# harryjfowen/PointsToWood

Measured on AMD Instinct MI355X. Metric: classified points/sec, higher is better.
Workload: dtype f16x3

## Files before the change

### include/p2w.h

```cpp
#ifndef P2W_H
#define P2W_H

#include <stddef.h>
#include <stdint.h>

#ifdef __cplusplus
extern "C" {
#endif

typedef void* p2w_stream_t;

#define P2W_OK 0
#define P2W_EINVAL (-1)
#define P2W_ENULL (-2)
#define P2W_EALIGN (-3)
#define P2W_EWORKSPACE (-4)
#define P2W_EUNSUPPORTED (-5)

#define P2W_MAX_K 64
#define P2W_MAX_K_WIDE 100
#define P2W_MAX_K_CONV 32

int32_t p2w_version(void);
const char* p2w_strerror(int32_t code);
// ... 170 lines not shown
    float* m;
    float* v;
    int64_t n;
} p2w_optim_tensor;
typedef struct p2w_optim_hyper {
    double lr, beta1, beta2, eps, weight_decay, max_norm, growth_factor, backoff_factor;
    int32_t growth_interval;
    int32_t scaling;
} p2w_optim_hyper;
typedef struct p2w_optim_state {
    double sumsq;
    float norm, coef;
    float inv_scale;
    float scale;
    int32_t found_inf;
    int32_t growth_tracker;
    int64_t t;
    int64_t skipped;
    float decay, omb1, beta2, omb2, step_size, rsb2, eps;
    int32_t reserved;
} p2w_optim_state;
size_t p2w_clip_adamw_ws_size(const int64_t* numel, int32_t T);
int32_t p2w_clip_adamw(const p2w_optim_tensor* tensors, int32_t T, const p2w_optim_hyper* hyper, p2w_optim_state* state, void* ws,
                       size_t ws_bytes, p2w_stream_t stream);

int32_t p2w_vote(const int32_t* nbr, const int32_t* deg, int32_t k, const float* pred, const float* prob, int32_t n,
                 float any_wood, float* label_out, float* pwood_out, p2w_stream_t stream);

int32_t p2w_tile_bbox(const float* xyzr, const int32_t* ptr, int32_t B, int32_t n_bound, float* bbox, p2w_stream_t stream);
int32_t p2w_tile_bbox_count(int32_t B, int32_t n_bound);


int32_t p2w_stem(const float* xyzr, int32_t n, const float* w, const float* b, int32_t C, float* out,
                 p2w_stream_t stream);

typedef struct p2w_epilogue {
    const float* bias;
    const float* sc0;
    const float* sh0;
    const float* sc1;
    const float* sh1;
    const float* residual;
    int32_t ldr;
    int32_t relu0, relu1, relu2, relu_final;
    uint32_t* range;
    const void* interp;
    int32_t interp_rows;
} p2w_epilogue;

#define P2W_RANGE_HI 6.0e4f
#define P2W_RANGE_LO 0.03125f
#define P2W_RANGE_SLOTS 16
#define P2W_RANGE_WORDS (64 * P2W_RANGE_SLOTS)

void p2w_packed_dims(int32_t N, int32_t K, int32_t* N_pad, int32_t* K_pad);

int32_t p2w_gemm(const float* A, int32_t lda, const float* Wp, int32_t M, int32_t N, int32_t K,
                 const p2w_epilogue* epi, float* out, int32_t ldo, p2w_stream_t stream);

int32_t p2w_sa_conv(const float* P, int32_t ldp, const float* xyzr_src, const int32_t* idx, const int32_t* batch_dst,
                    const float* sf, const int32_t* nbr, const int32_t* deg, int32_t kw, int32_t M,
                    const float* w1r4 , const float* W2p, int32_t C1, int32_t C2,
                    const float* b2, const float* bn_s, const float* bn_t, float* out, int32_t ldo,
                    p2w_stream_t stream);

#define P2W_PREC_F16X3 0
#define P2W_PREC_F16 1
#define P2W_PREC_BF16 2
int32_t p2w_packed_dims_h(int32_t prec, int32_t N, int32_t K, int32_t* N_pad, int32_t* K_pad);

#define P2W_GEMM_TILE_128 1
#define P2W_GEMM_TILE_256 2
#define P2W_GEMM_GENERIC_EPI 4
#define P2W_GEMM_ORDER_ROWS 8
#define P2W_GEMM_ORDER_COLS 16
#define P2W_GEMM_RESIDUAL_H 32
#define P2W_GEMM_STREAMK 64
#define P2W_GEMM_NO_STREAMK 128
#define P2W_GEMM_TILE_64 (1 << 24)
#define P2W_GEMM_NO_TILE_64 (1 << 25)
#define P2W_SA_ITEM_256 1
#define P2W_SA_ITEM_128 2
#define P2W_SA_PACK8 4

int32_t p2w_gemm_h2(int32_t prec, const void* A_h, int32_t ldh_a, const void* Wh, float wscale, int32_t M, int32_t N,
                    int32_t K, const p2w_epilogue* epi, float* out_f32, int32_t ldo, void* out_h, int32_t ldh_o,
                    int32_t flags, p2w_stream_t stream);
size_t p2w_gemm_h2_sk_ws_bytes(void);
int32_t p2w_gemm_h2_sk(int32_t prec, const void* A_h, int32_t ldh_a, const void* Wh, float wscale, int32_t M, int32_t N,
                       int32_t K, const p2w_epilogue* epi, float* out_f32, int32_t ldo, void* out_h, int32_t ldh_o,
                       void* ws, size_t ws_bytes, int32_t flags, p2w_stream_t stream);
size_t p2w_gemm_h2_rowdot_ws_bytes(int32_t M, int32_t N);
int32_t p2w_gemm_h2_rowdot(int32_t prec, const void* A_h, int32_t ldh_a, const void* Wh, float wscale, int32_t M, int32_t N,
                           int32_t K, const p2w_epilogue* epi, const float* dot_w, float dot_b, float* out, void* ws,
                           size_t ws_bytes, int32_t flags, p2w_stream_t stream);
size_t p2w_sa_conv_h_ws_bytes(int32_t M, int32_t flags);
int32_t p2w_sa_conv_h(int32_t prec, const float* P, int32_t ldp, int32_t n_src, const float* xyzr_src, const int32_t* idx,
                      const int32_t* batch_dst, const float* sf, const int32_t* nbr, const int32_t* deg, int32_t kw,
                      int32_t M, const float* w1r4, const void* W2h, float wscale, int32_t C1, int32_t C2,
                      const float* b2, const float* bn_s, const float* bn_t, float* out, int32_t ldo, void* out_h,
                      int32_t ldh, void* ws, size_t ws_bytes, int32_t flags, p2w_stream_t stream);
int32_t p2w_sa_conv_h_rows(int32_t prec, const float* P, int32_t ldp, int32_t n_src, const float* xyzr_src, const int32_t* idx,
                           const int32_t* batch_dst, const float* sf, const int32_t* nbr, const int32_t* deg, int32_t kw,
                           int32_t M, const float* w1r4, const void* W2h, float wscale, int32_t C1, int32_t C2,
                           const float* b2, const float* bn_s, const float* bn_t, float* out, int32_t ldo, void* out_h,
                           int32_t ldh, void* ws, size_t ws_bytes, int32_t flags, const int32_t* src_row, uint32_t* range,
                           p2w_stream_t stream);
int32_t p2w_stem_h2(int32_t prec, const float* xyzr, int32_t n, const float* w, const float* b, int32_t C, float* out,
                    void* out_h, int32_t ldh, uint32_t* range, p2w_stream_t stream);
int32_t p2w_stem_h2_indexed(int32_t prec, const float* xyzr, int32_t n, const float* w, const float* b, int32_t C, float* out,
                            void* out_h, int32_t ldh, uint32_t* range, p2w_stream_t stream);
int32_t p2w_interp_concat_h2(int32_t prec, const float* xc, int32_t Fc, const float* xyzr_c, const float* xyzr_f,
                             const int32_t* nbr, const int32_t* deg, int32_t kw, const float* skip, int32_t Fs, int32_t m,
                             void* out_h, int32_t ldh, p2w_stream_t stream);
int32_t p2w_interp_weights(const float* xyzr_c, const float* xyzr_f, const int32_t* nbr, const int32_t* deg, int32_t kw, int32_t m,
                           void* records, p2w_stream_t stream);
int32_t p2w_concat_xyz_h2(int32_t prec, const float* x, int32_t F, const float* xyzr, int32_t m, void* out_h, int32_t ldh,
                          p2w_stream_t stream);

int32_t p2w_interp_concat(const float* xc, int32_t Fc, const float* xyzr_c, const float* xyzr_f, const int32_t* nbr,
                          const int32_t* deg, int32_t kw, const float* skip, int32_t Fs, int32_t m, float* out,
                          int32_t ldo, p2w_stream_t stream);

int32_t p2w_concat_xyz(const float* x, int32_t F, const float* xyzr, int32_t m, float* out, int32_t ldo,
                       p2w_stream_t stream);

int32_t p2w_segment_max(const float* x, int32_t ldx, int32_t F, const int32_t* ptr, int32_t B, float* out,
                        p2w_stream_t stream);

int32_t p2w_rowdot(const float* x, int32_t ldx, int32_t F, const float* w, float b, int32_t m, float* out,
                   p2w_stream_t stream);

int32_t p2w_fill_batch_nbr(const int32_t* batch, int32_t m, int32_t* nbr, int32_t* deg, p2w_stream_t stream);


int32_t p2w_segment_max_arg(const float* x, int32_t ldx, int32_t F, const int32_t* ptr, int32_t B, float* out, int32_t* arg,
                            p2w_stream_t stream);
int32_t p2w_segment_max_bwd(const float* grad_out, int32_t ldg, const int32_t* arg, const int32_t* ptr, int32_t B, int32_t F,
                            float* grad_x, int32_t ldx, int32_t n, p2w_stream_t stream);
size_t p2w_interp_bwd_ws_bytes(int32_t m, int32_t kw, int32_t n_coarse);
int32_t p2w_interp_bwd(const float* grad_out, int32_t ldg, int32_t F, const float* xyzr_c, const float* xyzr_f, const int32_t* nbr,
                       const int32_t* deg, int32_t kw, int32_t m, int32_t n_coarse, float* grad_x, int32_t ldx, void* ws,
                       size_t ws_bytes, p2w_stream_t stream);

int32_t p2w_edge_l1(const float* P, int32_t ldp, const float* rec_src, const float* rec_dst, const int32_t* ptr, const int32_t* src,
                    const float* Wg, int32_t n_src, int32_t M, int32_t E, int32_t C1, float* geo, float* H1, int32_t ldh,
                    p2w_stream_t stream);
#define P2W_EDGE_CHUNK 1024
size_t p2w_edge_l1_bwd_ws_bytes(int32_t E, int32_t n_src, int32_t C1);
int32_t p2w_edge_l1_bwd(const float* gH, int32_t ldg, const float* H1, int32_t ldh, const float* geo, const int32_t* src,
                        const float* Wg, int32_t n_src, int32_t E, int32_t C1, float* gP, int32_t ldgp, float* gR, float* gWg, void* ws,
                        size_t ws_bytes, p2w_stream_t stream);

#define P2W_BN_GROUP 16
size_t p2w_relu_bn_max_ws_bytes(int32_t E, int32_t M, int32_t C2);
int32_t p2w_relu_bn_max(const float* z, int32_t ldz, const int32_t* ptr, const float* gamma, const float* beta, float* running_mean,
                        float* running_var, double momentum, double eps, int32_t E, int32_t M, int32_t C2, float* out, float* ext,
                        int32_t* arg, float* mean, float* invstd, void* ws, size_t ws_bytes, p2w_stream_t stream);
int32_t p2w_relu_bn_max_bwd(const float* g, const float* z, int32_t ldz, const int32_t* ptr, const int32_t* arg, const float* ext,
                            const float* mean, const float* invstd, const float* gamma, int32_t E, int32_t M, int32_t C2, float* dz,
                            int32_t lddz, float* dgamma, float* dbeta, void* ws, size_t ws_bytes, p2w_stream_t stream);

#define P2W_BN_CHAIN_MAX 3
#define P2W_BN_CHAIN_ROWS 32
typedef struct p2w_bn_stage {
    const float* dw_w;
// ... 98 lines not shown
```

### pointstowood_amd/_lib.py

```python
from __future__ import annotations

import ctypes as C
import os

import torch

_HERE = os.path.dirname(os.path.abspath(__file__))
LIB_PATH = os.path.join(_HERE, "libp2w_gfx950.so")

_vp, _i32, _f32, _sz = C.c_void_p, C.c_int32, C.c_float, C.c_size_t


class Epilogue(C.Structure):
    _fields_ = [("bias", _vp), ("sc0", _vp), ("sh0", _vp), ("sc1", _vp), ("sh1", _vp), ("residual", _vp),
                ("ldr", _i32), ("relu0", _i32), ("relu1", _i32), ("relu2", _i32), ("relu_final", _i32), ("range", _vp),
                ("interp", _vp), ("interp_rows", _i32)]


class BnStage(C.Structure):
    _fields_ = [("dw_w", _vp), ("dw_b", _vp), ("gamma", _vp), ("beta", _vp), ("running_mean", _vp), ("running_var", _vp),
                ("momentum", C.c_double), ("eps", C.c_double), ("relu", _i32)]


class OptimTensor(C.Structure):
    _fields_ = [("p", _vp), ("g", _vp), ("m", _vp), ("v", _vp), ("n", C.c_int64)]


class OptimHyper(C.Structure):
    _fields_ = [(k, C.c_double) for k in ("lr", "beta1", "beta2", "eps", "weight_decay", "max_norm", "growth_factor", "backoff_factor")] + \
               [("growth_interval", _i32), ("scaling", _i32)]


class OptimState(C.Structure):
    _fields_ = [("sumsq", C.c_double), ("norm", _f32), ("coef", _f32), ("inv_scale", _f32), ("scale", _f32), ("found_inf", _i32),
                ("growth_tracker", _i32), ("t", C.c_int64), ("skipped", C.c_int64), ("decay", _f32), ("omb1", _f32), ("beta2", _f32),
                ("omb2", _f32), ("step_size", _f32), ("rsb2", _f32), ("eps", _f32), ("reserved", _i32)]


SEARCH_X_INDEX_IN_W, SEARCH_Q_ROW_IN_W, SEARCH_BOX = 1, 2, 4
PREC_F16X3, PREC_F16, PREC_BF16 = 0, 1, 2
PREC_OF = {"f16x3": PREC_F16X3, "fp16": PREC_F16, "bf16": PREC_BF16}
GEMM_TILE_128, GEMM_TILE_256, GEMM_GENERIC_EPI, GEMM_ORDER_ROWS, GEMM_ORDER_COLS, GEMM_RESIDUAL_H = 1, 2, 4, 8, 16, 32
GEMM_STREAMK, GEMM_NO_STREAMK = 64, 128
SA_ITEM_256, SA_ITEM_128, SA_PACK8 = 1, 2, 4
CLUSTER_LINK, CLUSTER_COMPRESS, CLUSTER_NUMBER, CLUSTER_ALL = 1, 2, 4, 7
MAX_K_WIDE = 100
EVAL_CHUNK, EVAL_MAX_CLASSES = 4096, 8
LOSS_CHUNK = 4096
EDGE_CHUNK = 1024
BN_GROUP = 16
BN_CHAIN_MAX, BN_CHAIN_ROWS = 3, 32
FEED_CHUNK, FEED_STREAM = 256, 0x50325746
SAMPLE_STREAM, SAMPLE_TILE, SAMPLE_N_MAX = 0x50325753, 1024, 1 << 24
CAP_STREAM, CAP_N_MAX, CAP_S_MAX, CAP_OUT_MAX = 0x50325743, 1 << 30, 1 << 20, 1 << 38
OPTIM_CHUNK, OPTIM_GROUP, OPTIM_MAX_TENSORS = 4096, 32, 4096
F32, F16, BF16 = 0, 1, 2

SIGNATURES = {
    "p2w_version": (_i32, []),
    "p2w_strerror": (C.c_char_p, [_i32]),
    "p2w_pack_xyzr": (_i32, [_vp, _i32, _vp, _vp, _i32, _i32, _vp, _vp, _vp]),
    "p2w_voxel_sample_ws_bytes": (_sz, [_i32]),
    "p2w_voxel_sample": (_i32, [_vp, _vp, _i32, _i32, _f32, _vp, _vp, _vp, _vp, _vp, _vp, _vp, _vp, _vp, _vp, _sz, _vp]),
    "p2w_voxel_sample_table_ws_bytes": (_sz, [_i32, C.c_int64]),
    "p2w_voxel_sample_table": (_i32, [_vp, _vp, _i32, _i32, _f32, _vp, _vp, _vp, _vp, _vp, _vp, _vp, _vp, _vp, _vp, _vp, _vp, C.c_int64,
                                      _vp, _sz, _vp]),
    "p2w_voxel_sample_table_prepare": (_i32, [_vp, _sz, _vp]),
    "p2w_voxel_sample_table_prepared": (_i32, [_vp, _vp, _i32, _i32, _f32, _vp, _vp, _vp, _vp, _vp, _vp, _vp, _vp, _vp, _vp, _vp, _vp, C.c_int64,
                                               _vp, _sz, _vp]),
    "p2w_knn_grid_indexed": (_i32, [_vp, _vp, _vp, _vp, _vp, _vp, _vp, _vp, _i32, _i32, _i32, _vp, _vp, _vp, _i32, _vp]),
    "p2w_ball_query_grid_indexed": (_i32, [_vp, _vp, _vp, _vp, _vp, _vp, _vp, _vp, _i32, _i32, C.c_double, _i32, _vp, _vp, _i32, _vp]),
    "p2w_knn_hint2": (_i32, [_vp, _vp, _vp, _i32, _i32, _vp, _vp, _vp]),
    "p2w_knn_grid": (_i32, [_vp, _vp, _vp, _vp, _vp, _vp, _vp, _i32, _i32, _i32, _vp, _vp, _vp, _i32, _vp]),
    "p2w_ball_query_grid": (_i32, [_vp, _vp, _vp, _vp, _vp, _vp, _vp, _i32, _i32, C.c_double, _i32, _vp, _vp, _i32, _vp]),
    "p2w_index_records": (_i32, [_vp, _vp, _vp, _i32, _i32, _vp, _vp]),
    "p2w_voxel_grid": (_i32, [_vp, _vp, _i32, _i32, _f32, _vp, _vp, _sz, _vp]),
    "p2w_consecutive_cluster": (_i32, [_vp, _i32, _vp, _vp, _vp, _vp, _sz, _vp]),
    "p2w_level_gather": (_i32, [_vp, _vp, _vp, _vp, _i32, _i32, _vp, _vp, _vp]),
    "p2w_ball_query": (_i32, [_vp, _vp, _vp, _vp, _vp, _i32, _i32, C.c_double, _i32, _vp, _vp, _vp, _i32, _vp]),
    "p2w_knn": (_i32, [_vp, _vp, _vp, _vp, _vp, _i32, _i32, _i32, _vp, _vp, _vp, _i32, _vp]),
    "p2w_morton_order_ws_bytes": (_sz, [_i32]),
    "p2w_morton_order": (_i32, [_vp, _i32, _vp, _vp, _vp, _sz, _vp]),
    "p2w_cells_nd": (_i32, [_vp, _i32, _i32, _i32, _f32, _vp, _vp, _sz, _vp]),
    "p2w_sort_pairs_u64_ws_bytes": (_sz, [_i32]),
    "p2w_sort_pairs_u64": (_i32, [_vp, _vp, _vp, _vp, _i32, _vp, _sz, _vp]),
    "p2w_key_runs_ws_bytes": (_sz, [_i32]),
    "p2w_key_runs": (_i32, [_vp, _i32, _i32, _vp, _vp, _vp, _vp, _sz, _vp]),
    "p2w_knn_refine_f64": (_i32, [_vp, _vp, _vp, _vp, _vp, _vp, C.c_double, C.c_double, C.c_double, _vp, _i32, _i32, _i32, _vp, _vp, _vp]),
    "p2w_cell_starts_ws_bytes": (_sz, [C.c_int64]),
    "p2w_cell_starts": (_i32, [_vp, _i32, C.c_int64, _vp, _vp, _sz, _vp]),
    "p2w_vote": (_i32, [_vp, _vp, _i32, _vp, _vp, _i32, _f32, _vp, _vp, _vp]),
    "p2w_euclid_cluster_ws_bytes": (_sz, [C.c_int64]),
    "p2w_euclid_cluster": (_i32, [_vp, _vp, _vp, _vp, _vp, C.c_int64, C.c_double, C.c_int64, C.c_int64, _i32, _vp, _vp, _vp, _vp, _sz, _vp]),
    "p2w_knn_wide_f64": (_i32, [_vp, _vp, _vp, _vp, _vp, C.c_int64, _i32, C.c_double, _vp, _vp]),
    "p2w_pathlen_grow_ws_bytes": (_sz, [C.c_int64]),
    "p2w_pathlen_grow": (_i32, [_vp, _vp, C.c_int64, _i32, _i32, _i32, C.c_double, C.c_double, C.c_double, _vp, _vp, C.c_int64, _vp, _vp,
                                _vp, _sz, _vp]),
    "p2w_pathlen_sssp_ws_bytes": (_sz, [C.c_int64, C.c_int64]),
    "p2w_pathlen_sssp": (_i32, [_vp, _vp, C.c_int64, C.c_int64, _i32, _vp, _vp, _vp, _vp, _sz, _vp]),
    "p2w_pathlen_weights": (_i32, [_vp, _vp, C.c_int64, _vp, _vp]),
    "p2w_confusion_ws_bytes": (_sz, [C.c_int64, _i32, _i32]),
    "p2w_confusion": (_i32, [_vp, _vp, _vp, _vp, C.c_int64, _i32, _i32, _vp, _vp, _vp, _vp, _sz, _vp]),
    "p2w_poly1_focal_ws_bytes": (_sz, [C.c_int64]),
    "p2w_poly1_focal": (_i32, [_vp, _vp, _vp, C.c_int64, C.c_int64, C.c_double, C.c_double, C.c_double, C.c_double, C.c_double, _vp, _vp, _vp,
                               _vp, _sz, _vp]),
    "p2w_train_feed_ws_size": (_sz, [C.c_int64, _i32]),
    "p2w_train_feed": (_i32, [_vp, _vp, _vp, C.c_int64, _i32, _vp, _vp, _i32, C.c_int64, _vp, C.c_uint64, C.c_uint32, _vp, _vp, _vp, _vp,
                              _vp, _vp, _vp, _vp, _vp, _sz, _vp]),
    "p2w_random_subset_ws_size": (_sz, [C.c_int64]),
    "p2w_random_subset": (_i32, [C.c_int64, C.c_int64, C.c_uint64, C.c_uint32, C.c_uint32, _vp, _vp, _vp, _vp, _sz, _vp]),
    "p2w_cap_subset_ws_size": (_sz, [C.c_int64, C.c_int64]),
    "p2w_cap_subset": (_i32, [C.c_int64, _vp, _vp, C.c_int64, C.c_int64, _vp, _vp, C.c_uint64, C.c_uint32, C.c_uint32, _vp, _vp, _vp, _vp,
                              _sz, _vp]),
    "p2w_clip_adamw_ws_size": (_sz, [_vp, _i32]),
    "p2w_clip_adamw": (_i32, [C.POINTER(OptimTensor), _i32, C.POINTER(OptimHyper), _vp, _vp, _sz, _vp]),
    "p2w_tile_bbox": (_i32, [_vp, _vp, _i32, _i32, _vp, _vp]),
    "p2w_tile_bbox_count": (_i32, [_i32, _i32]),
    "p2w_stem": (_i32, [_vp, _i32, _vp, _vp, _i32, _vp, _vp]),
    "p2w_packed_dims": (None, [_i32, _i32, C.POINTER(_i32), C.POINTER(_i32)]),
    "p2w_gemm": (_i32, [_vp, _i32, _vp, _i32, _i32, _i32, C.POINTER(Epilogue), _vp, _i32, _vp]),
    "p2w_sa_conv": (_i32, [_vp, _i32, _vp, _vp, _vp, _vp, _vp, _vp, _i32, _i32, _vp, _vp, _i32, _i32, _vp, _vp, _vp,
                           _vp, _i32, _vp]),
    "p2w_packed_dims_h": (_i32, [_i32, _i32, _i32, C.POINTER(_i32), C.POINTER(_i32)]),
    "p2w_gemm_h2": (_i32, [_i32, _vp, _i32, _vp, _f32, _i32, _i32, _i32, C.POINTER(Epilogue), _vp, _i32, _vp, _i32, _i32, _vp]),
    "p2w_gemm_h2_sk_ws_bytes": (_sz, []),
    "p2w_gemm_h2_sk": (_i32, [_i32, _vp, _i32, _vp, _f32, _i32, _i32, _i32, C.POINTER(Epilogue), _vp, _i32, _vp, _i32, _vp, _sz, _i32, _vp]),
    "p2w_gemm_h2_rowdot_ws_bytes": (_sz, [_i32, _i32]),
# ... 150 lines not shown
```

### pointstowood_amd/csrc/p2w_hgemm.h

```cpp
#pragma once
#include "p2w_common.h"
#include <type_traits>

typedef float f32x16 __attribute__((ext_vector_type(16)));
typedef _Float16 h8 __attribute__((ext_vector_type(8)));
typedef __bf16 bf8 __attribute__((ext_vector_type(8)));
typedef __fp16 hpair __attribute__((ext_vector_type(2)));
typedef _Float16 hpairn __attribute__((ext_vector_type(2)));
typedef __bf16 bpair __attribute__((ext_vector_type(2)));
typedef float fpair __attribute__((ext_vector_type(2)));
typedef __attribute__((address_space(3))) void* lds_vp;
typedef const __attribute__((address_space(1))) void* glb_vp;

constexpr int H_BK = 32;
constexpr int SA_EPI_COLS = 1024;

template <int PREC> struct HCfg {
    static constexpr int planes = PREC == 0 ? 2 : 1;
    static constexpr int kslab = PREC == 0 ? 32 : 64;
    static constexpr int kalign = PREC == 0 ? 32 : 64;
};

template <int PREC>
__device__ __forceinline__ f32x16 h_mfma(h8 a, h8 b, f32x16 c) {
// ... 1070 lines not shown
        Vals vb;
        gather(mb, k_of(c2), vb);
        meta_of(c3, mc);
        Degs dg_n;
        load_deg(c1.mt, dg_n);
        WRegs wk;
        load_w(k_of(c1), wk);
        __builtin_amdgcn_sched_barrier(0);
        if (g + 1 < total)
            issue((g + 1) & 1, W2h + (size_t)c1.nt * BN * NP * C1pad, c1.s * H_BK);
        const char* st = S + (size_t)(g & 1) * STAGE_CH * 16;
        h8 afq[2][NP][RT], bfq[2][NP][2];
#pragma unroll
        for (int kk = 0; kk < 2; ++kk)
#pragma unroll
            for (int p = 0; p < NP; ++p) {
#pragma unroll
                for (int t = 0; t < RT; ++t) afq[kk][p][t] = *reinterpret_cast<const h8*>(st + (offA[t] ^ (kk << 5) ^ (p << 6)));
#pragma unroll
                for (int t = 0; t < 2; ++t) bfq[kk][p][t] = *reinterpret_cast<const h8*>(st + (offB[t] ^ (kk << 5) ^ (p << 6)));
            }
#pragma unroll
        for (int kk = 0; kk < 2; ++kk) {
            auto& af = afq[kk];
            auto& bf = bfq[kk];
#pragma unroll
            for (int i = 0; i < RT; ++i)
#pragma unroll
                for (int j = 0; j < 2; ++j) {
                    if constexpr (PREC == 0) {
                        acc[i][j] = h_mfma<PREC>(af[1][i], bf[0][j], acc[i][j]);
                        acc[i][j] = h_mfma<PREC>(af[0][i], bf[1][j], acc[i][j]);
                    }
                    acc[i][j] = h_mfma<PREC>(af[0][i], bf[0][j], acc[i][j]);
                }
            if (kk == 0) {
                produce((g + 1) & 1, ma, k_of(c1), va, wk);
                constexpr int NM = 2 * RT * (PREC == 0 ? 3 : 1);
#pragma unroll
                for (int q = 0; q < NM; ++q) {
                    __builtin_amdgcn_sched_group_barrier(0x008, 1, 0);
                    __builtin_amdgcn_sched_group_barrier(0x002, (PREC == 0 ? 16 : 40) * NR / RT, 0);
                }
                __builtin_amdgcn_sched_barrier(0);
            }
        }
#pragma unroll
        for (int u = 0; u < NR; ++u) {
            asm volatile("" : "+v"(vb.v[u][0].x), "+v"(vb.v[u][0].y), "+v"(vb.v[u][0].z), "+v"(vb.v[u][0].w),
                              "+v"(vb.v[u][1].x), "+v"(vb.v[u][1].y), "+v"(vb.v[u][1].z), "+v"(vb.v[u][1].w));
            asm volatile("" : "+v"(mc.j[u]), "+v"(mc.g[u].x), "+v"(mc.g[u].y), "+v"(mc.g[u].z), "+v"(mc.g[u].w));
        }
#pragma unroll
        for (int i = 0; i < RT; ++i)
#pragma unroll
            for (int q = 0; q < GPT; ++q) asm volatile("" : "+v"(dg_n.d[i][q]));
        __builtin_amdgcn_s_waitcnt(p2w_vmcnt_imm(0));
        if (c0.s == nslab - 1) {
            SaEpiRegs<RT, GPT> e;
#pragma unroll
            for (int j = 0; j < 2; ++j) {
                const int col = min(c0.nt * BN + wc * 64 + j * 32 + (lane & 31), C2 - 1);
                e.bias[j] = Ep[col]; e.s[j] = Ep[SA_EPI_COLS + col]; e.t[j] = Ep[2 * SA_EPI_COLS + col];
            }
#pragma unroll
            for (int i = 0; i < RT; ++i)
#pragma unroll
                for (int q = 0; q < GPT; ++q) e.dsc[i][q] = (c0.mt * (BM / 32) + wr * RT + i >= M) ? -1 : dg_.d[i][q];
            sa_epilogue_regs<PREC, RT, G>(acc, wscale, c0.nt * BN, wc, lane, e, C2, out, ldo, out_h2, ldh, amax);
#pragma unroll
            for (int i = 0; i < RT; ++i)
#pragma unroll
                for (int j = 0; j < 2; ++j)
#pragma unroll
                    for (int e2 = 0; e2 < 16; ++e2) acc[i][j][e2] = 0.f;
        }
        __builtin_amdgcn_sched_barrier(0);
        va = vb; ma = mb; mb = mc; dg_ = dg_n;
        c0 = c1; c1 = c2; c2 = c3; c3 = nxt(c3);
    }
    if (range) range_commit_max(range, amax, lane);
}


__global__ __launch_bounds__(256) void sa_edge_meta_kernel(const float4* __restrict__ xyzr, const int* __restrict__ idx, const int* __restrict__ batch_dst,
                                    const float* __restrict__ sf, const int* __restrict__ nbr, const int* __restrict__ deg, int kw,
                                    int M, int n_src, int ldp4, int G, const int* __restrict__ list, const int* __restrict__ n_list_dev,
                                    const int* __restrict__ src_row, int* __restrict__ meta_j, float4* __restrict__ meta_g, int* __restrict__ desc,
                                    float4* __restrict__ zero_row);
constexpr int SA_PART_BLOCK = 1024;
__global__ __launch_bounds__(SA_PART_BLOCK) void sa_part_count_kernel(const int* __restrict__ deg, int kw, int M, int* __restrict__ blk_small);
__global__ __launch_bounds__(1024) void sa_part_scan_kernel(int* __restrict__ blk_small, int nblk, int M, int* __restrict__ counts);
__global__ __launch_bounds__(SA_PART_BLOCK) void sa_part_scatter_kernel(const int* __restrict__ deg, int kw, int M, const int* __restrict__ blk_small,
                                                                     int* __restrict__ list_small, int* __restrict__ list_large);

struct SaWs {
    float4 *mg_l, *mg_s;
    int *mj_l, *mj_s, *desc_l, *desc_s;
    int *list_s, *list_l, *blk, *counts;
    long t32, t8, nblk;
};
static inline SaWs sa_conv_carve(P2wArena& a, long M, int flags) {
    const bool pack8 = (flags & P2W_SA_PACK8) != 0;
    SaWs W = {};
    W.t32 = M;
    W.t8 = pack8 ? (M + 3) / 4 : 0;
    W.nblk = pack8 ? (M + SA_PART_BLOCK - 1) / SA_PART_BLOCK : 0;
    W.mg_l = a.take<float4>((size_t)W.t32 * 32, 16);
    W.mg_s = a.take<float4>((size_t)W.t8 * 32, 16);
    W.mj_l = a.take<int>((size_t)W.t32 * 32, 4);
    W.mj_s = a.take<int>((size_t)W.t8 * 32, 4);
    W.desc_l = a.take<int>((size_t)W.t32, 4);
    W.desc_s = a.take<int>((size_t)W.t8 * 4, 4);
    if (!pack8) { a.raw(256, 1); return W; }
    W.list_s = a.take<int>((size_t)M, 4);
    W.list_l = a.take<int>((size_t)M, 4);
    W.blk = a.take<int>((size_t)W.nblk, 4);
    W.counts = a.take<int>(16, 4);
    a.raw(1024, 1);
    return W;
}

template <int PREC>
static int32_t launch_sa_conv_h(const float* P, int32_t ldp, int32_t n_src, const float* xyzr_src, const int32_t* idx, const int32_t* batch_dst,
                                const float* sf, const int32_t* nbr, const int32_t* deg, int32_t kw, int32_t M,
                                const float* w1r4, const _Float16* W2h, float wscale, int32_t C1, int32_t C2, const float* b2,
                                const float* bn_s, const float* bn_t, float* out, int32_t ldo, _Float16* out_h2, int32_t ldh,
                                void* ws, size_t ws_bytes, int32_t flags, hipStream_t stream, const int32_t* src_row = nullptr,
                                unsigned* range = nullptr) {
    constexpr int KA = HCfg<PREC>::kalign;
    const int C2pad = (C2 + 255) / 256 * 256, C1pad = (C1 + KA - 1) / KA * KA;
    if (C1pad > 512 || C2 > SA_EPI_COLS || (long)M >= (1L << 25) || ((long)n_src + 1) * (ldp / 4) >= (1L << 31)) return P2W_EUNSUPPORTED;
    if (ldp < C1pad) return P2W_EINVAL;
    P2wArena arena(ws);
    const SaWs L = sa_conv_carve(arena, M, flags);
    if (ws == nullptr || ws_bytes < arena.bytes()) return P2W_EWORKSPACE;
    if (reinterpret_cast<uintptr_t>(ws) & 15u) return P2W_EALIGN;
    const int n_cu = p2w_cu_count();
    const bool wide = (flags & (P2W_SA_ITEM_256 | P2W_SA_ITEM_128)) ? (flags & P2W_SA_ITEM_256) != 0 : C2 > 128;
    const int tpi = wide ? 4 : 8, nNt3 = p2w_cdiv(C2, wide ? 256 : 128);
    const float4* x4 = reinterpret_cast<const float4*>(xyzr_src);
    auto run = [&](auto g_c, const int* list, const int* n_list_dev, const int* tiles_dev, long tiles_max, float4* meta_g, int* meta_j,
                   int* desc) {
        constexpr int G = decltype(g_c)::value;
        const long rows_max = tiles_max * 32;
        sa_edge_meta_kernel<<<p2w_cdiv(rows_max, 256), 256, 0, stream>>>(x4, idx, batch_dst, sf, nbr, deg, kw, M, n_src, ldp / 4, G,
                                                                       list, n_list_dev, src_row, meta_j, meta_g, desc,
                                                                       reinterpret_cast<float4*>(const_cast<float*>(P) + (size_t)n_src * ldp));
        const long items = p2w_cdiv(tiles_max, tpi) * nNt3;
        int grid = (int)(items < n_cu ? items : n_cu);
        if (grid >= 8) grid &= ~7;
        const int nMt3 = (int)p2w_cdiv(tiles_max, tpi);
        if (wide)
            sa_conv16p_kernel<PREC, 256, 2, G><<<grid, 512, 0, stream>>>(
                P, ldp, meta_j, meta_g, desc, tiles_dev, (int)tiles_max, w1r4, C1, C1pad, W2h, (size_t)C2pad * C1pad, wscale, C2, nMt3,
                nNt3, b2, bn_s, bn_t, out, ldo, out_h2, ldh, range);
        else
            sa_conv16p_kernel<PREC, 128, 2, G><<<grid, 512, 0, stream>>>(
                P, ldp, meta_j, meta_g, desc, tiles_dev, (int)tiles_max, w1r4, C1, C1pad, W2h, (size_t)C2pad * C1pad, wscale, C2, nMt3,
                nNt3, b2, bn_s, bn_t, out, ldo, out_h2, ldh, range);
    };
    if (!(flags & P2W_SA_PACK8)) {
        run(std::integral_constant<int, 32>{}, nullptr, nullptr, nullptr, M, L.mg_l, L.mj_l, L.desc_l);
        return P2W_LAUNCH_STATUS();
    }
    int* counts = L.counts;
    sa_part_count_kernel<<<(int)L.nblk, SA_PART_BLOCK, 0, stream>>>(deg, kw, M, L.blk);
    sa_part_scan_kernel<<<1, 1024, 0, stream>>>(L.blk, (int)L.nblk, M, counts);
    sa_part_scatter_kernel<<<(int)L.nblk, SA_PART_BLOCK, 0, stream>>>(deg, kw, M, L.blk, L.list_s, L.list_l);
    run(std::integral_constant<int, 8>{}, L.list_s, counts + 0, counts + 2, L.t8, L.mg_s, L.mj_s, L.desc_s);
    run(std::integral_constant<int, 32>{}, L.list_l, counts + 1, counts + 3, L.t32, L.mg_l, L.mj_l, L.desc_l);
    return P2W_LAUNCH_STATUS();
}

int32_t p2w_gemm_h1_impl(int32_t prec, const _Float16* Ah, int32_t ldh_a, const _Float16* Wp, float wscale, int32_t M, int32_t N,
                         int32_t K, const EpiArgs& ep, float* out_f32, int32_t ldo, _Float16* out_h2, int32_t ldh_o,
                         int32_t flags, hipStream_t stream, const float* dotw = nullptr, float* part = nullptr, int32_t ldpart = 0,
                         float* skws = nullptr, size_t skws_bytes = 0);
int32_t p2w_sa_conv_h1_impl(int32_t prec, const float* P, int32_t ldp, int32_t n_src, const float* xyzr_src, const int32_t* idx,
                            const int32_t* batch_dst, const float* sf, const int32_t* nbr, const int32_t* deg, int32_t kw,
                            int32_t M, const float* w1r4, const _Float16* W2h, float wscale, int32_t C1, int32_t C2,
                            const float* b2, const float* bn_s, const float* bn_t, float* out, int32_t ldo, _Float16* out_h2,
                            int32_t ldh, void* ws, size_t ws_bytes, int32_t flags, hipStream_t stream, const int32_t* src_row = nullptr,
                            unsigned* range = nullptr);
```

Baseline: 20.95 million.

## Add dedicated f16x3 SA conv kernel for small first-layer channel counts

```diff
diff --git a/include/p2w.h b/include/p2w.h
--- a/include/p2w.h
+++ b/include/p2w.h
@@ -276,6 +276,7 @@
 #define P2W_SA_ITEM_256 1
 #define P2W_SA_ITEM_128 2
 #define P2W_SA_PACK8 4
+#define P2W_SA_LEGACY_L1 8
 
 int32_t p2w_gemm_h2(int32_t prec, const void* A_h, int32_t ldh_a, const void* Wh, float wscale, int32_t M, int32_t N,
                     int32_t K, const p2w_epilogue* epi, float* out_f32, int32_t ldo, void* out_h, int32_t ldh_o,
diff --git a/pointstowood_amd/_lib.py b/pointstowood_amd/_lib.py
--- a/pointstowood_amd/_lib.py
+++ b/pointstowood_amd/_lib.py
@@ -42,7 +42,7 @@
 PREC_OF = {"f16x3": PREC_F16X3, "fp16": PREC_F16, "bf16": PREC_BF16}
 GEMM_TILE_128, GEMM_TILE_256, GEMM_GENERIC_EPI, GEMM_ORDER_ROWS, GEMM_ORDER_COLS, GEMM_RESIDUAL_H = 1, 2, 4, 8, 16, 32
 GEMM_STREAMK, GEMM_NO_STREAMK = 64, 128
-SA_ITEM_256, SA_ITEM_128, SA_PACK8 = 1, 2, 4
+SA_ITEM_256, SA_ITEM_128, SA_PACK8, SA_LEGACY_L1 = 1, 2, 4, 8
 CLUSTER_LINK, CLUSTER_COMPRESS, CLUSTER_NUMBER, CLUSTER_ALL = 1, 2, 4, 7
 MAX_K_WIDE = 100
 EVAL_CHUNK, EVAL_MAX_CLASSES = 4096, 8
diff --git a/pointstowood_amd/csrc/p2w_hgemm.h b/pointstowood_amd/csrc/p2w_hgemm.h
--- a/pointstowood_amd/csrc/p2w_hgemm.h
+++ b/pointstowood_amd/csrc/p2w_hgemm.h
@@ -1176,6 +1176,155 @@
     if (range) range_commit_max(range, amax, lane);
 }
 
+constexpr int SA_L1_WAVES = 4, SA_L1_WG_PER_CU = 2;
+template <int PREC, int G, int NSLAB>
+__global__ __launch_bounds__(64 * SA_L1_WAVES, SA_L1_WG_PER_CU) void sa_conv_l1_kernel(const float* __restrict__ P, const int* __restrict__ meta_j,
+                                                                         const float4* __restrict__ meta_g, const int* __restrict__ desc,
+                                                                         const int* __restrict__ tiles_dev, int M, const float* __restrict__ w1r4,
+                                                                         const _Float16* __restrict__ W2h, float wscale, int C2,
+                                                                         const float* __restrict__ b2, const float* __restrict__ bn_s,
+                                                                         const float* __restrict__ bn_t, float* __restrict__ out, int ldo,
+                                                                         _Float16* __restrict__ out_h2, int ldh, unsigned* __restrict__ range) {
+    static_assert(PREC == 0, "f16x3 only: the single-plane precisions stay on sa_conv16p_kernel");
+    constexpr int GPT = 32 / G, C1PAD = H_BK * NSLAB, NK = 2 * NSLAB, NT = 64 * SA_L1_WAVES;
+    constexpr int SLAB_B = 128 * 128;
+    if (tiles_dev) M = *tiles_dev;
+    if (M <= 0) return;
+    __shared__ __attribute__((aligned(16))) char S[NSLAB * SLAB_B + 4 * C1PAD * 4 + 3 * 128 * 4];
+    float* const Wr = reinterpret_cast<float*>(S + NSLAB * SLAB_B);
+    float* const Ep = Wr + 4 * C1PAD;
+    const int tid = threadIdx.x, lane = tid & 63, r = lane & 31, h = lane >> 5;
+    const int wave = __builtin_amdgcn_readfirstlane(tid >> 6);
+    auto img = [](int row, int chunk) { return (row * 8 + (chunk ^ ((row >> 1) & 7))) * 16; };
+    int vb = blockIdx.x;
+    if ((gridDim.x & 7) == 0) vb = (blockIdx.x & 7) * (gridDim.x >> 3) + (blockIdx.x >> 3);
+    const long long ngrp = (M + SA_L1_WAVES - 1) / SA_L1_WAVES;
+    const int g0 = (int)(ngrp * vb / gridDim.x), g1 = (int)(ngrp * (vb + 1) / gridDim.x);
+    const int t_end = min(g1 * SA_L1_WAVES, M);
+    int t = g0 * SA_L1_WAVES + wave;
+
+    struct Meta { int j; float4 g; };
+    struct Vals { float4 v[NK][2]; };
+    const float4* const P4 = reinterpret_cast<const float4*>(P);
+    auto load_meta = [&](int tile, Meta& m, int (&d)[GPT]) {
+        const int tc = min(tile, M - 1), row = tc * 32 + r;
+        m.j = meta_j[row];
+        m.g = meta_g[row];
+#pragma unroll
+        for (int q = 0; q < GPT; ++q) d[q] = desc[tc * GPT + q];
+    };
+    auto gather = [&](const Meta& m, int kq, Vals& dst) {
+        const float4* p = P4 + ((unsigned)m.j + (unsigned)(4 * kq + 2 * h));
+        dst.v[kq][0] = p[0];
+        dst.v[kq][1] = p[1];
+    };
+    Meta mc, mn;
+    int dc[GPT], dn[GPT];
+    load_meta(t, mc, dc);
+    load_meta(t + SA_L1_WAVES, mn, dn);
+    constexpr int NPC = NSLAB * 1024 / NT;
+    uint4 wp[NPC];
+#pragma unroll
+    for (int u = 0; u < NPC; ++u) {
+        const int i = tid + u * NT, c = i & 7, row = (i >> 3) & 127, s = i >> 10;
+        wp[u] = *reinterpret_cast<const uint4*>(W2h + (size_t)row * (2 * C1PAD) + 64 * s + 8 * c);
+    }
+    static_assert(4 * C1PAD <= NT && 128 <= NT, "one table element per thread");
+    const int iw = min(tid, 4 * C1PAD - 1), ie = min(tid, C2 - 1);
+    const float w1v = w1r4[iw], e0 = b2[ie], e1 = bn_s[ie], e2 = bn_t[ie];
+    Vals vc;
+#pragma unroll
+    for (int kq = 0; kq < NK; ++kq) gather(mc, kq, vc);
+#pragma unroll
+    for (int u = 0; u < NPC; ++u) {
+        const int i = tid + u * NT, c = i & 7, row = (i >> 3) & 127, s = i >> 10;
+        *reinterpret_cast<uint4*>(S + s * SLAB_B + img(row, c)) = wp[u];
+    }
+    Wr[iw] = w1v;
+    Ep[ie] = e0; Ep[128 + ie] = e1; Ep[256 + ie] = e2;
+#pragma unroll
+    for (int kq = 0; kq < NK; ++kq)
+        asm volatile("" : "+v"(vc.v[kq][0].x), "+v"(vc.v[kq][0].y), "+v"(vc.v[kq][0].z), "+v"(vc.v[kq][0].w),
+                          "+v"(vc.v[kq][1].x), "+v"(vc.v[kq][1].y), "+v"(vc.v[kq][1].z), "+v"(vc.v[kq][1].w));
+    asm volatile("" : "+v"(mn.j), "+v"(mn.g.x), "+v"(mn.g.y), "+v"(mn.g.z), "+v"(mn.g.w));
+    asm volatile("" : "+v"(mc.g.x), "+v"(mc.g.y), "+v"(mc.g.z), "+v"(mc.g.w));
+    __syncthreads();
+
+    float amax = 0.f;
+    if (t < t_end) {
+        const int offB = img(r, h);
+        for (; t < t_end; t += SA_L1_WAVES) {
+            Meta mnn;
+            int dnn[GPT];
+            load_meta(t + 2 * SA_L1_WAVES, mnn, dnn);
+            f32x16 acc[2][1][2];
+#pragma unroll
+            for (int c = 0; c < 2; ++c)
+#pragma unroll
+                for (int j = 0; j < 2; ++j)
+#pragma unroll
+                    for (int e = 0; e < 16; ++e) acc[c][0][j][e] = 0.f;
+            const float gx = mc.g.x, gy = mc.g.y, gz = mc.g.z, gw = mc.g.w;
+#pragma unroll
+            for (int kq = 0; kq < NK; ++kq) {
+                const int k = 16 * kq + 8 * h;
+                unsigned hiw[4], low[4];
+#pragma unroll
+                for (int half = 0; half < 2; ++half) {
+                    const float* w = Wr + k + 4 * half;
+                    const float4 wx = *reinterpret_cast<const float4*>(w), wy = *reinterpret_cast<const float4*>(w + C1PAD),
+                                 wz = *reinterpret_cast<const float4*>(w + 2 * C1PAD), wf = *reinterpret_cast<const float4*>(w + 3 * C1PAD);
+                    const float4 p = vc.v[kq][half];
+                    float v[4];
+                    v[0] = fmaxf(fmaf(gw, wf.x, fmaf(gz, wz.x, fmaf(gy, wy.x, fmaf(gx, wx.x, p.x)))), 0.f);
+                    v[1] = fmaxf(fmaf(gw, wf.y, fmaf(gz, wz.y, fmaf(gy, wy.y, fmaf(gx, wx.y, p.y)))), 0.f);
+                    v[2] = fmaxf(fmaf(gw, wf.z, fmaf(gz, wz.z, fmaf(gy, wy.z, fmaf(gx, wx.z, p.z)))), 0.f);
+                    v[3] = fmaxf(fmaf(gw, wf.w, fmaf(gz, wz.w, fmaf(gy, wy.w, fmaf(gx, wx.w, p.w)))), 0.f);
+                    split_pair(v[0], v[1], hiw[2 * half], low[2 * half]);
+                    split_pair(v[2], v[3], hiw[2 * half + 1], low[2 * half + 1]);
+                }
+                gather(mn, kq, vc);
+                __builtin_amdgcn_sched_barrier(0);
+                typedef unsigned u32x4 __attribute__((ext_vector_type(4)));
+                const h8 a_hi = __builtin_bit_cast(h8, u32x4{hiw[0], hiw[1], hiw[2], hiw[3]});
+                const h8 a_lo = __builtin_bit_cast(h8, u32x4{low[0], low[1], low[2], low[3]});
+                const char* st = S + (kq >> 1) * SLAB_B;
+                const int ob = offB ^ ((kq & 1) << 5);
+#pragma unroll
+                for (int c = 0; c < 4; ++c) {
+                    const h8 b_hi = *reinterpret_cast<const h8*>(st + 4096 * c + ob);
+                    const h8 b_lo = *reinterpret_cast<const h8*>(st + 4096 * c + (ob ^ 64));
+                    f32x16& a = acc[c >> 1][0][c & 1];
+                    a = h_mfma<PREC>(a_lo, b_hi, a);
+                    a = h_mfma<PREC>(a_hi, b_lo, a);
+                    a = h_mfma<PREC>(a_hi, b_hi, a);
+                }
+            }
+#pragma unroll
+            for (int kq = 0; kq < NK - 1; ++kq)
+                asm volatile("" : "+v"(vc.v[kq][0].x), "+v"(vc.v[kq][0].y), "+v"(vc.v[kq][0].z), "+v"(vc.v[kq][0].w),
+                                  "+v"(vc.v[kq][1].x), "+v"(vc.v[kq][1].y), "+v"(vc.v[kq][1].z), "+v"(vc.v[kq][1].w));
+            asm volatile("" : "+v"(mnn.j), "+v"(mnn.g.x), "+v"(mnn.g.y), "+v"(mnn.g.z), "+v"(mnn.g.w));
+#pragma unroll
+            for (int wc = 0; wc < 2; ++wc) {
+                SaEpiRegs<1, GPT> e;
+#pragma unroll
+                for (int j = 0; j < 2; ++j) {
+                    const int col = min(wc * 64 + j * 32 + r, C2 - 1);
+                    e.bias[j] = Ep[col]; e.s[j] = Ep[128 + col]; e.t[j] = Ep[256 + col];
+                }
+#pragma unroll
+                for (int q = 0; q < GPT; ++q) e.dsc[0][q] = t >= M ? -1 : dc[q];
+                sa_epilogue_regs<PREC, 1, G>(acc[wc], wscale, 0, wc, lane, e, C2, out, ldo, out_h2, ldh, amax);
+            }
+            mc = mn; mn = mnn;
+#pragma unroll
+            for (int q = 0; q < GPT; ++q) { dc[q] = dn[q]; dn[q] = dnn[q]; }
+        }
+    }
+    if (range) range_commit_max(range, amax, lane);
+}
+
 
 __global__ __launch_bounds__(256) void sa_edge_meta_kernel(const float4* __restrict__ xyzr, const int* __restrict__ idx, const int* __restrict__ batch_dst,
                                     const float* __restrict__ sf, const int* __restrict__ nbr, const int* __restrict__ deg, int kw,
@@ -1241,6 +1390,20 @@
         sa_edge_meta_kernel<<<p2w_cdiv(rows_max, 256), 256, 0, stream>>>(x4, idx, batch_dst, sf, nbr, deg, kw, M, n_src, ldp / 4, G,
                                                                        list, n_list_dev, src_row, meta_j, meta_g, desc,
                                                                        reinterpret_cast<float4*>(const_cast<float*>(P) + (size_t)n_src * ldp));
+        if constexpr (PREC == 0) {
+            if (!(flags & P2W_SA_LEGACY_L1) && !wide && C1pad <= 64 && C2 <= 128) {
+                const long wgs = p2w_cdiv(tiles_max, SA_L1_WAVES);
+                int grid = (int)(wgs < (long)n_cu * SA_L1_WG_PER_CU ? wgs : (long)n_cu * SA_L1_WG_PER_CU);
+                if (grid >= 8) grid &= ~7;
+                auto go = [&](auto ns) {
+                    sa_conv_l1_kernel<PREC, G, decltype(ns)::value><<<grid, 64 * SA_L1_WAVES, 0, stream>>>(
+                        P, meta_j, meta_g, desc, tiles_dev, (int)tiles_max, w1r4, W2h, wscale, C2, b2, bn_s, bn_t, out, ldo, out_h2, ldh, range);
+                };
+                if (C1pad <= 32) go(std::integral_constant<int, 1>{});
+                else go(std::integral_constant<int, 2>{});
+                return;
+            }
+        }
         const long items = p2w_cdiv(tiles_max, tpi) * nNt3;
         int grid = (int)(items < n_cu ? items : n_cu);
         if (grid >= 8) grid &= ~7;
```

After: 21.20 million, median of 6. 1.01x the previous value.
